# jermp/sshash

Measured on AMD Instinct MI355X. Metric: k-mer Lookups/sec (batched random queries, bit-exact ids), higher is better.
Workload: dtype u64

## Files before the change

sshash_amd/csrc/replica.hpp:

```cpp
#pragma once

#include <algorithm>
#include <atomic>

#include <cstdio>
#include <cstdlib>

#include <hip/hip_runtime.h>

#include <functional>
#include <mutex>
#include <stdexcept>
#include <string>
#include <unordered_map>
#include <vector>

#include "lookup_device.hpp"
#include "mphf_build.hpp"

namespace sshash_amd {

inline void hip_check(hipError_t e, char const* what) {
    if (e != hipSuccess) throw error(error_kind::hip, std::string("HIP error in ") + what + ": " + hipGetErrorString(e));
}
#define HIP_CHECK(x) ::sshash_amd::hip_check((x), #x)

struct device_guard {
    int prev = 0;
    int target;
    explicit device_guard(int dev) : target(dev) {
        HIP_CHECK(hipGetDevice(&prev));
        if (prev != dev) HIP_CHECK(hipSetDevice(dev));
    }
    ~device_guard() {
        if (prev != target) (void)hipSetDevice(prev);
    }
};

struct host_lane {
    hipStream_t stream = nullptr;
    void* pinned = nullptr;
    void* device = nullptr;
    size_t capacity = 0;
};

struct stream_block {
    void* block = nullptr;
    size_t bytes = 0;
    void free_block() {
        if (block) HIP_CHECK(hipFree(block));
        block = nullptr;
        bytes = 0;
    }
    void release() {
        if (block) (void)hipFree(block);
        block = nullptr;
        bytes = 0;
    }
};

template <typename Slot, size_t MAX_STREAMS, size_t MAX_BYTES>
class stream_cache {
public:
    Slot& get(void* stream, size_t bytes, size_t headroom) {
        std::lock_guard<std::mutex> lock(m_mutex);
        auto it = m_slots.try_emplace(stream).first;
        it->second.last_use = ++m_clock;
        Slot& slot = it->second.slot;
        if (slot.bytes >= bytes) return slot;
        slot.free_block();
        const size_t want = bytes + bytes / headroom + 4096;
        size_t held = want;
        for (auto const& kv : m_slots) held += kv.second.slot.bytes;
        while (m_slots.size() > 1 && (m_slots.size() > MAX_STREAMS || held > MAX_BYTES)) {
            auto oldest = m_slots.end();
            for (auto jt = m_slots.begin(); jt != m_slots.end(); ++jt)
                if (jt != it && (oldest == m_slots.end() || jt->second.last_use < oldest->second.last_use)) oldest = jt;
            held -= oldest->second.slot.bytes;
            oldest->second.slot.release();
            m_slots.erase(oldest);
        }
        HIP_CHECK(hipMalloc(&slot.block, want));
        slot.bytes = want;
        return slot;
    }
    void release(void* stream) {
        std::lock_guard<std::mutex> lock(m_mutex);
        auto it = m_slots.find(stream);
        if (it == m_slots.end()) return;
        it->second.slot.release();
        m_slots.erase(it);
    }
    void clear() {
        std::lock_guard<std::mutex> lock(m_mutex);
        for (auto& kv : m_slots) kv.second.slot.release();
        m_slots.clear();
    }

private:
    struct entry {
        Slot slot;
        uint64_t last_use = 0;
    };
    std::mutex m_mutex;
    std::unordered_map<void*, entry> m_slots;
    uint64_t m_clock = 0;
};

struct device_replica {
    int device = -1;
    uint64_t bytes = 0;
    uint64_t bytes_still_to_come = 0;
    dict_view view{};
    skew_part_dev* d_skew = nullptr;
    uint64_t directory_overflowed = 0;
    uint64_t directory_entries = 0;
    uint64_t sk_keys = 0, sk_heavy_keys = 0, sk_heavy_kmers = 0, sk_unplaced = 0, sk_slots_used = 0, sk_bytes = 0;
    uint32_t sk_absent_reason = 1;
    uint64_t sk_histogram[20] = {0};
    std::vector<void*> allocations;
    hipMemPool_t scratch_pool = nullptr;
    void create_scratch_pool() {
        hipMemPoolProps props{};
        props.allocType = hipMemAllocationTypePinned;
        props.handleTypes = hipMemHandleTypeNone;
        props.location.type = hipMemLocationTypeDevice;
        props.location.id = device;
        if (hipMemPoolCreate(&scratch_pool, &props) != hipSuccess) {
            scratch_pool = nullptr;
            (void)hipGetLastError();
            if (std::getenv("SSHASH_AMD_VERBOSE"))
                fprintf(stderr, "[sshash_amd] device %d: no private memory pool (hipMemPoolCreate failed): stream-ordered scratch comes out of the default pool\n", device);
            return;
        }
        uint64_t keep = ~uint64_t(0);
        (void)hipMemPoolSetAttribute(scratch_pool, hipMemPoolAttrReleaseThreshold, &keep);
    }
    void* stream_alloc(size_t bytes, hipStream_t s) const {
        void* p = nullptr;
        if (scratch_pool) HIP_CHECK(hipMallocFromPoolAsync(&p, bytes ? bytes : 8, scratch_pool, s));
        else HIP_CHECK(hipMallocAsync(&p, bytes ? bytes : 8, s));
        return p;
    }

    mutable std::mutex launch_mutex;
    struct stream_scratch : stream_block {
        hipStream_t aux = nullptr;
        hipEvent_t first_done[2] = {nullptr, nullptr};
        hipEvent_t tail_done[2] = {nullptr, nullptr};
        void free_block() {
            if (aux) HIP_CHECK(hipStreamSynchronize(aux));
            stream_block::free_block();
        }
        void release() {
            if (aux) (void)hipStreamSynchronize(aux);
            for (int i = 0; i < 2; ++i) {
                if (first_done[i]) (void)hipEventDestroy(first_done[i]);
                if (tail_done[i]) (void)hipEventDestroy(tail_done[i]);
                first_done[i] = tail_done[i] = nullptr;
            }
            if (aux) (void)hipStreamDestroy(aux);
            aux = nullptr;
            stream_block::release();
        }
    };
    mutable stream_cache<stream_scratch, 16, ~size_t(0)> queue_scratch;
    mutable stream_cache<stream_block, 64, size_t(8) << 30> read_scratch;
    stream_scratch& scratch_for(void* stream, size_t bytes, bool with_aux_stream) const {
        stream_scratch& slot = queue_scratch.get(stream, bytes, 4);
        if (with_aux_stream && !slot.aux) {
            HIP_CHECK(hipStreamCreateWithFlags(&slot.aux, hipStreamNonBlocking));
            for (int i = 0; i < 2; ++i) {
                HIP_CHECK(hipEventCreateWithFlags(&slot.first_done[i], hipEventDisableTiming));
                HIP_CHECK(hipEventCreateWithFlags(&slot.tail_done[i], hipEventDisableTiming));
            }
        }
        return slot;
    }
    void* read_scratch_for(void* stream, size_t bytes) const { return read_scratch.get(stream, bytes, 8).block; }

    void release_stream_scratch(void* stream) const {
        queue_scratch.release(stream);
        read_scratch.release(stream);
    }

    mutable std::mutex lanes_mutex;
    mutable std::vector<host_lane*> idle_lanes;
    host_lane* acquire_lane(size_t bytes) const;
    void release_lane(host_lane* lane) const;

    template <typename T>
    T* put(std::vector<T> const& v) {
        T* d = nullptr;
        const size_t n = (v.empty() ? 1 : v.size()) * sizeof(T);
        HIP_CHECK(hipMalloc(&d, n));
        allocations.push_back(d);
        if (!v.empty()) HIP_CHECK(hipMemcpy(d, v.data(), v.size() * sizeof(T), hipMemcpyHostToDevice));
        bytes += n;
        return d;
    }
    mphf_view put_mphf(mphf_host const& f) {
        mphf_view v = f.view();
        v.parts = put(f.parts);
        v.pilots = put(f.pilots);
        v.free_slots = put(f.free_slots);
        return v;
    }
    device_replica() = default;
    device_replica(device_replica const&) = delete;
    device_replica& operator=(device_replica const&) = delete;
    ~device_replica() {
        if (device < 0) return;
        int prev = 0;
        if (hipGetDevice(&prev) != hipSuccess) return;
        (void)hipSetDevice(device);
        for (void* p : allocations) (void)hipFree(p);
        if (scratch_pool) {
            (void)hipDeviceSynchronize();
            (void)hipMemPoolDestroy(scratch_pool);
        }
        queue_scratch.clear();
        read_scratch.clear();
        for (host_lane* lane : idle_lanes) {
            if (lane->pinned) (void)hipHostFree(lane->pinned);
            if (lane->device) (void)hipFree(lane->device);
            if (lane->stream) (void)hipStreamDestroy(lane->stream);
            delete lane;
        }
        (void)hipSetDevice(prev);
    }
};

struct own_stream {
    device_replica const* rep;
    hipStream_t s = nullptr;
    explicit own_stream(device_replica const* r) : rep(r) { HIP_CHECK(hipStreamCreateWithFlags(&s, hipStreamNonBlocking)); }
    own_stream(own_stream const&) = delete;
    own_stream& operator=(own_stream const&) = delete;
    ~own_stream() {
        (void)hipStreamSynchronize(s);
        rep->release_stream_scratch(s);
        (void)hipStreamDestroy(s);
    }
};

class device_buffers {
public:
    device_buffers() = default;
    device_buffers(device_replica const* rep, hipStream_t s) : m_rep(rep), m_stream(s) {}
    device_buffers(device_buffers const&) = delete;
    device_buffers& operator=(device_buffers const&) = delete;
    ~device_buffers() {
        for (void* p : m_owned) free_one(p);
    }
    template <typename T>
    T* alloc(uint64_t n) {
        const size_t bytes = std::max<uint64_t>(n * sizeof(T), 8);
        void* p = nullptr;
        if (m_rep) p = m_rep->stream_alloc(bytes, m_stream);
        else HIP_CHECK(hipMalloc(&p, bytes));
        m_owned.push_back(p);
        return static_cast<T*>(p);
    }
    void release(void const* p) {
        for (void*& q : m_owned)
            if (q == p) {
                free_one(q);
                q = nullptr;
            }
    }
    void keep(void const* p, device_replica& rep) {
        for (void*& q : m_owned)
            if (q == p) {
                rep.allocations.push_back(q);
                q = nullptr;
            }
    }

private:
    void free_one(void* p) const {
        if (!p) return;
        if (m_rep) (void)hipFreeAsync(p, m_stream);
        else (void)hipFree(p);
    }
    device_replica const* m_rep = nullptr;
    hipStream_t m_stream = nullptr;
    std::vector<void*> m_owned;
};

class engine;

std::vector<int> resident_devices(engine const& eng);

void run_lanes(engine const& eng, std::vector<int> const& devices, size_t bytes, std::function<void(size_t, int, host_lane&)> const& fn,
               std::atomic<bool>* failed = nullptr);

}
```

sshash_amd/csrc/streaming.hip:

```cpp
#include <hip/hip_runtime.h>
#include <sys/stat.h>

#include <algorithm>
#include <atomic>
#include <cstring>
#include <exception>
#include <stdexcept>
#include <thread>

#include "engine.hpp"
#include "hooks.hpp"
#include "reads.hpp"
#include "replica.hpp"

namespace sshash_amd {

namespace {

template <int W, bool CANON>
__device__ __forceinline__ hit_t seed_lookup(dict_view const& d, skew_part_dev const* __restrict__ skew,
                                             kmer_w<W> const& x, kmer_w<W> const& x_rc, minimizer_t mf, minimizer_t mr) {
    if constexpr (CANON) {
        if (mf.value < mr.value) return probe_canonical<W, true>(d, skew, x, x_rc, mf);
        if (mr.value < mf.value) return probe_canonical<W, true>(d, skew, x, x_rc, mr);
        hit_t h = probe_canonical<W, true>(d, skew, x, x_rc, mf);
        if (!h.found) h = probe_canonical<W, true>(d, skew, x, x_rc, mr);
        return h;
    } else {
        hit_t h = probe_regular<W, true>(d, skew, x, mf);
        if (!h.found) {
            const bool mf_found = h.minimizer_found;
            h = probe_regular<W, true>(d, skew, x_rc, mr);
            h.orientation = -1;
            h.minimizer_found = h.minimizer_found || mf_found;
        }
        return h;
    }
}

__device__ __forceinline__ uint64_t wave_sum(uint64_t v) {
    for (int o = 32; o > 0; o >>= 1) v += __shfl_down(v, o, 64);
    return v;
}

__device__ __forceinline__ void block_report(uint64_t c_kmers, uint64_t c_invalid, uint64_t c_negative, uint64_t c_searches,
                                             uint64_t c_extensions, uint64_t* __restrict__ report) {
    __shared__ uint64_t partial[4][5];
    c_kmers = wave_sum(c_kmers);
    c_invalid = wave_sum(c_invalid);
    c_negative = wave_sum(c_negative);
    c_searches = wave_sum(c_searches);
    c_extensions = wave_sum(c_extensions);
    if ((threadIdx.x & 63) == 0) {
        uint64_t* mine = partial[threadIdx.x >> 6];
        mine[0] = c_kmers;
        mine[1] = c_invalid;
        mine[2] = c_negative;
        mine[3] = c_searches;
        mine[4] = c_extensions;
    }
    __syncthreads();
    if (threadIdx.x != 0) return;
    uint64_t t[5];
    for (int j = 0; j < 5; ++j) t[j] = partial[0][j] + partial[1][j] + partial[2][j] + partial[3][j];
    if (t[0] == 0) return;
    atomicAdd(reinterpret_cast<unsigned long long*>(report + 0), (unsigned long long)t[0]);
    atomicAdd(reinterpret_cast<unsigned long long*>(report + 1), (unsigned long long)(t[3] + t[4]));
    atomicAdd(reinterpret_cast<unsigned long long*>(report + 2), (unsigned long long)t[2]);
    atomicAdd(reinterpret_cast<unsigned long long*>(report + 3), (unsigned long long)t[1]);
    atomicAdd(reinterpret_cast<unsigned long long*>(report + 4), (unsigned long long)t[3]);
    atomicAdd(reinterpret_cast<unsigned long long*>(report + 5), (unsigned long long)t[4]);
}


__global__ void __launch_bounds__(256)
stream_pack_kernel(const char* __restrict__ bases, const uint64_t total_bases, uint16_t* __restrict__ packed, uint8_t* __restrict__ okay) {
    const uint64_t t = uint64_t(blockIdx.x) * blockDim.x + threadIdx.x;
    const uint64_t at = 8 * t;
    if (at >= total_bases) return;
    uint64_t v = 0;
    if (at + 8 <= total_bases && ((reinterpret_cast<uintptr_t>(bases) + at) & 7) == 0) {
        v = *reinterpret_cast<const uint64_t*>(bases + at);
    } else {
        for (uint32_t b = 0; b < 8 && at + b < total_bases; ++b) v |= uint64_t(uint8_t(bases[at + b])) << (8 * b);
    }
    uint64_t two = (v >> 1) & 0x0303030303030303ULL;
    two = (two | (two >> 6)) & 0x000F000F000F000FULL;
    two = (two | (two >> 12)) & 0x000000FF000000FFULL;
    two = two | (two >> 24);
    const uint64_t u = v & 0xDFDFDFDFDFDFDFDFULL;
    auto nonzero = [](uint64_t z) { return ((z & 0x7F7F7F7F7F7F7F7FULL) + 0x7F7F7F7F7F7F7F7FULL) | z; };
    uint64_t ok = ~(nonzero(u ^ 0x4141414141414141ULL) & nonzero(u ^ 0x4343434343434343ULL) & nonzero(u ^ 0x4747474747474747ULL) &
                    nonzero(u ^ 0x5454545454545454ULL)) & 0x8080808080808080ULL;
    ok >>= 7;
    ok |= ok >> 7;
    ok |= ok >> 14;
    ok |= ok >> 28;
    packed[t] = uint16_t(two);
    okay[t] = uint8_t(ok);
}

__device__ __forceinline__ uint64_t first_invalid_base(const uint64_t* __restrict__ okay, uint64_t from, uint64_t end) {
    uint64_t p = from;
    while (p < end) {
        const uint64_t bad = ~okay[p >> 6] >> (p & 63u);
        if (bad) {
            p += uint64_t(__builtin_ctzll(bad));
            break;
        }
        p = (p | 63u) + 1;
    }
    return p < end ? p : end;
}

__device__ __forceinline__ uint64_t first_valid_base(const uint64_t* __restrict__ okay, uint64_t from, uint64_t end) {
    uint64_t p = from;
    while (p < end) {
        const uint64_t good = okay[p >> 6] >> (p & 63u);
        if (good) {
            p += uint64_t(__builtin_ctzll(good));
            break;
        }
        p = (p | 63u) + 1;
    }
    return p < end ? p : end;
}

__device__ __forceinline__ uint64_t read_bases32(const uint64_t* __restrict__ packed, uint64_t p) {
    const uint64_t i = p >> 5;
    return funnel_shr(packed[i], packed[i + 1], 2 * (uint32_t(p) & 31u));
}

template <int W>
__device__ __forceinline__ void string_bases32(dict_view const& d, uint64_t p, uint64_t& bases, uint64_t& marks) {
    const uint32_t rel = uint32_t(p) & 31u;
    if constexpr (W == 1) {
        const uint4* A = reinterpret_cast<const uint4*>(d.granules) + 2 * (p >> 5);
        const uint4 q0 = A[0], q1 = A[1];
        bases = funnel_shr(uint64_t(q0.x) | (uint64_t(q0.y) << 32), uint64_t(q0.z) | (uint64_t(q0.w) << 32), 2 * rel);
        marks = (uint64_t(q1.x) | (uint64_t(q1.y) << 32)) >> rel;
    } else {
        const uint4* G = reinterpret_cast<const uint4*>(d.granules) + (p >> 5);
        const uint4 g0 = G[0], g1 = G[1];
        bases = funnel_shr(uint64_t(g0.z) | (uint64_t(g0.w) << 32), uint64_t(g1.z) | (uint64_t(g1.w) << 32), 2 * rel);
        marks = (uint64_t(g0.y) | (uint64_t(g1.y) << 32)) >> rel;
    }
}

struct run_step_t {
    uint64_t s, marks, read;
    uint32_t have;
};

template <int W>
__device__ __forceinline__ run_step_t run_step_load(dict_view const& d, const uint64_t* __restrict__ packed, uint64_t off, bool forward,
                                                    uint64_t b, uint64_t run) {
    run_step_t t;
    const uint64_t top = off - run;
    t.have = forward || top >= 32 ? 32u : uint32_t(top);
    string_bases32<W>(d, forward ? off + d.k + run : top - t.have, t.s, t.marks);
    t.read = read_bases32(packed, b + run);
    return t;
}

__device__ __forceinline__ uint32_t run_step_length(run_step_t const& t, bool forward) {
    const uint64_t along = forward ? t.s : revcomp_word(t.s << ((2 * (32 - t.have)) & 63u));
    const uint64_t diff = along ^ t.read;
    const uint32_t same = diff ? uint32_t(__builtin_ctzll(diff)) >> 1 : 32u;
    const uint32_t gate = forward ? uint32_t(__brev(uint32_t(t.marks))) : uint32_t((t.marks >> 1) << (32 - t.have));
    const uint32_t inside = gate ? uint32_t(__builtin_clz(gate)) : 32u;
    const uint32_t step = same < inside ? same : inside;
    return step < t.have ? step : t.have;
}

template <int W>
__device__ __forceinline__ uint64_t extend_run(dict_view const& d, const uint64_t* __restrict__ packed, uint64_t off, int ori, uint64_t b,
                                               uint64_t room, run_step_t t) {
    const bool forward = ori > 0;
    uint64_t run = 0;
    for (;;) {
        uint64_t step = run_step_length(t, forward);
        if (step > room - run) step = room - run;
        run += step;
        if (step < 32 || run >= room) break;
        t = run_step_load<W>(d, packed, off, forward, b, run);
    }
    return run;
}

__device__ __forceinline__ void row_flush(uint64_t* __restrict__ row, bool partial, uint32_t& c_invalid, uint32_t& c_negative, uint32_t& c_searches,
                                          uint32_t& c_extensions) {
    const uint64_t s = c_searches, e = c_extensions;
    if (partial) {
        row[1] += s + e;
        row[2] += c_negative;
        row[3] += c_invalid;
        row[4] += s;
        row[5] += e;
    } else {
        row[1] = s + e;
        row[2] = c_negative;
        row[3] = c_invalid;
        row[4] = s;
        row[5] = e;
    }
    c_invalid = c_negative = c_searches = c_extensions = 0;
}

#ifndef SSHASH_STREAM_WAVES
#define SSHASH_STREAM_WAVES 5
#endif
enum : int { STREAM_TOTALS = 0, STREAM_ROWS = 1, STREAM_RUN_COUNTS = 2, STREAM_RUN_RECORDS = 3, STREAM_COVER = 4 };

__device__ __forceinline__ void run_record_store(dict_view const& d, run_sink const& sink, const uint64_t* __restrict__ offsets, uint64_t r,
                                                 uint64_t cursor, uint64_t at, uint64_t off, uint32_t sid, int ori, uint64_t n) {
    if (cursor >= sink.capacity || cursor >= sink.run_offsets[r + 1]) return;
    const uint64_t kmer_id = off - uint64_t(sid) * (d.k - 1), in_string = off - d.endpoints[sid];
    const uint32_t read_pos = uint32_t(at - offsets[r]), length = uint32_t(n) | (ori > 0 ? 0u : 0x80000000u);
    uint4* const rec = static_cast<uint4*>(sink.records) + 2 * cursor;
    rec[0] = make_uint4(uint32_t(kmer_id), uint32_t(kmer_id >> 32), sid, 0u);
    rec[1] = make_uint4(uint32_t(in_string), uint32_t(in_string >> 32), read_pos, length);
}

__device__ __forceinline__ void cover_mark(uint64_t* __restrict__ cover, uint64_t lo, uint64_t hi) {
    const uint64_t w0 = lo >> 6, w1 = (hi - 1) >> 6;
    const unsigned long long first = ~0ULL << (lo & 63u), last = ~0ULL >> (63u - (uint32_t(hi - 1) & 63u));
    unsigned long long* const words = reinterpret_cast<unsigned long long*>(cover);
    if (w0 == w1) {
        (void)__hip_atomic_fetch_or(words + w0, first & last, __ATOMIC_RELAXED, __HIP_MEMORY_SCOPE_AGENT);
        return;
    }
    (void)__hip_atomic_fetch_or(words + w0, first, __ATOMIC_RELAXED, __HIP_MEMORY_SCOPE_AGENT);
    for (uint64_t w = w0 + 1; w < w1; ++w) words[w] = ~0ULL;
    (void)__hip_atomic_fetch_or(words + w1, last, __ATOMIC_RELAXED, __HIP_MEMORY_SCOPE_AGENT);
}

__device__ __forceinline__ void cover_mark_run(dict_view const& d, run_sink const& sink, uint64_t off, uint32_t sid, int ori, uint64_t n) {
    const uint64_t kmer_id = off - uint64_t(sid) * (d.k - 1);
    const uint64_t lo = ori > 0 ? kmer_id : kmer_id + 1 - n;
    cover_mark(static_cast<uint64_t*>(sink.records), lo, lo + n);
}

template <int W, bool CANON, bool SK, int MODE>
__global__ void __launch_bounds__(256, SSHASH_STREAM_WAVES)
streaming_run_kernel(const dict_view d, const skew_part_dev* __restrict__ skew, const uint64_t* __restrict__ packed,
                     const uint64_t* __restrict__ okay, const uint64_t* __restrict__ offsets, const uint64_t n_reads,
                     const uint64_t reads_per_wave, const uint32_t move_out_every, uint64_t* __restrict__ report, const run_sink sink) {
    constexpr bool PER_READ = MODE == STREAM_ROWS, COUNT_RUNS = MODE == STREAM_RUN_COUNTS, RECORDS = MODE == STREAM_RUN_RECORDS, COVER = MODE == STREAM_COVER;
    __shared__ uint4 stage[SK ? 4 * 256 : 1];
    uint4* const wave_stage = stage + (SK ? (threadIdx.x >> 6) * 256 : 0);
    __shared__ unsigned long long moved_out[4][5];
    uint32_t c_invalid = 0, c_negative = 0, c_searches = 0, c_extensions = 0;
// ... 288 lines not shown
                        }
                    }
                }
            }
        }
        const bool finishing = live && !walking;
        STAT(st_full, finishing && !settled);
        if (finishing && !settled) {
            const minimizer_t mf = compute_minimizer<W>(x, k, d.m, d.hash_magic);
            const minimizer_t mr = compute_minimizer<W>(x_rc, k, d.m, d.hash_magic);
            if (!SK && neg_unknown_mini && mf.value == prev_f && mr.value == prev_r) {
                found = false;
            } else {
                prev_f = mf.value;
                prev_r = mr.value;
                const hit_t h = seed_lookup<W, CANON>(d, skew, x, x_rc, mf, mr);
                found = h.found;
                off = h.kmer_offset;
                ori = h.orientation;
                if constexpr (RECORDS || COVER) hit_sid = h.string_id;
                neg_unknown_mini = !SK && !h.found && !h.minimizer_found;
            }
        }
        if (finishing) {
            if (found) {
                ++c_searches;
                neg_unknown_mini = false;
                pending = cur + 1 + k <= valid_end;
                if constexpr (COUNT_RUNS) ++n_runs;
                if constexpr (RECORDS) {
                    if (!pending) {
                        run_record_store(d, sink, offsets, wave_first + my_row, cursor, cur, off, hit_sid, ori, 1);
                        ++cursor;
                    }
                }
                if constexpr (COVER) {
                    if (!pending) cover_mark_run(d, sink, off, hit_sid, ori, 1);
                }
            } else {
                ++c_negative;
            }
            ++cur;
        }
    }
#ifdef SSHASH_STREAM_STATS
    const unsigned long long st_neg_kept = wave_sum(st_kept_lane);
    if (lane == 0 && MODE == STREAM_TOTALS) {
        unsigned long long* st = reinterpret_cast<unsigned long long*>(report) + 6;
        atomicAdd(st + 0, st_turns); atomicAdd(st + 1, st_fresh); atomicAdd(st + 2, st_walk); atomicAdd(st + 3, st_ext); atomicAdd(st + 4, st_slot1);
        atomicAdd(st + 5, st_inv); atomicAdd(st + 6, st_idle); atomicAdd(st + 7, st_full); atomicAdd(st + 8, st_neg_kept); atomicAdd(st + 9, st_short);
    }
#endif
    if constexpr (PER_READ) {
        if (my_row != ROW_NONE) row_flush(wave_rows + uint64_t(my_row & ~ROW_PARTIAL) * 6, (my_row & ROW_PARTIAL) != 0, c_invalid, c_negative, c_searches, c_extensions);
    } else if constexpr (!RECORDS) {
        if constexpr (COUNT_RUNS) {
            if (my_row != ROW_NONE) sink.run_offsets[wave_first + my_row] = n_runs;
        }
        const bool first = lane == 0;
        block_report(first ? wave_moved_out[4] : 0, uint64_t(c_invalid) + (first ? wave_moved_out[0] : 0), uint64_t(c_negative) + (first ? wave_moved_out[1] : 0),
                     uint64_t(c_searches) + (first ? wave_moved_out[2] : 0), uint64_t(c_extensions) + (first ? wave_moved_out[3] : 0), report);
    }
}

__global__ void __launch_bounds__(256)
stream_rows_sum_kernel(const uint64_t* __restrict__ rows, const uint64_t n_reads, uint64_t* __restrict__ report) {
    uint64_t c_kmers = 0, c_invalid = 0, c_negative = 0, c_searches = 0, c_extensions = 0;
    const uint64_t stride = uint64_t(gridDim.x) * blockDim.x;
    for (uint64_t r = uint64_t(blockIdx.x) * blockDim.x + threadIdx.x; r < n_reads; r += stride) {
        const uint64_t* row = rows + 6 * r;
        c_kmers += row[0];
        c_negative += row[2];
        c_invalid += row[3];
        c_searches += row[4];
        c_extensions += row[5];
    }
    block_report(c_kmers, c_invalid, c_negative, c_searches, c_extensions, report);
}

constexpr uint32_t SCAN_PER_LANE = 16, SCAN_TILE = 256 * SCAN_PER_LANE;
inline uint64_t scan_tiles(uint64_t n) { return (n + SCAN_TILE - 1) / SCAN_TILE; }

__device__ __forceinline__ uint64_t block_exclusive_scan(uint64_t v, uint64_t& total) {
    __shared__ uint64_t wave_total[4];
    const uint32_t lane = threadIdx.x & 63u, w = threadIdx.x >> 6;
    uint64_t inc = v;
    for (uint32_t o = 1; o < 64; o <<= 1) {
        const uint64_t t = __shfl_up(inc, o, 64);
        if (lane >= o) inc += t;
    }
    __syncthreads();
    if (lane == 63) wave_total[w] = inc;
    __syncthreads();
    uint64_t before = 0;
    total = 0;
    for (uint32_t j = 0; j < 4; ++j) {
        if (j < w) before += wave_total[j];
        total += wave_total[j];
    }
    return before + inc - v;
}

__global__ void __launch_bounds__(256)
scan_tile_sums_kernel(const uint64_t* __restrict__ data, const uint64_t n, uint64_t* __restrict__ sums) {
    const uint64_t base = uint64_t(blockIdx.x) * SCAN_TILE + threadIdx.x * SCAN_PER_LANE;
    uint64_t v = 0;
    for (uint32_t j = 0; j < SCAN_PER_LANE; ++j)
        if (base + j < n) v += data[base + j];
    uint64_t total;
    block_exclusive_scan(v, total);
    if (threadIdx.x == 0) sums[blockIdx.x] = total;
}

__global__ void __launch_bounds__(256)
scan_sums_kernel(uint64_t* __restrict__ sums, const uint64_t tiles) {
    uint64_t carry = 0;
    for (uint64_t at = 0; at < tiles; at += 256) {
        const uint64_t i = at + threadIdx.x;
        const uint64_t v = i < tiles ? sums[i] : 0;
        uint64_t total;
        const uint64_t before = block_exclusive_scan(v, total);
        if (i < tiles) sums[i] = carry + before;
        carry += total;
    }
}

__global__ void __launch_bounds__(256)
scan_apply_kernel(uint64_t* __restrict__ data, const uint64_t n, const uint64_t* __restrict__ sums) {
    const uint64_t base = uint64_t(blockIdx.x) * SCAN_TILE + threadIdx.x * SCAN_PER_LANE;
    uint64_t e[SCAN_PER_LANE], v = 0;
#pragma unroll
    for (uint32_t j = 0; j < SCAN_PER_LANE; ++j) {
        e[j] = base + j < n ? data[base + j] : 0;
        v += e[j];
    }
    uint64_t total;
    uint64_t at = sums[blockIdx.x] + block_exclusive_scan(v, total);
#pragma unroll
    for (uint32_t j = 0; j < SCAN_PER_LANE; ++j) {
        if (base + j < n) data[base + j] = at;
        at += e[j];
    }
}

void exclusive_scan_u64(uint64_t* data, uint64_t n, uint64_t* sums, hipStream_t s) {
    if (n == 0) return;
    const uint64_t tiles = scan_tiles(n);
    hipLaunchKernelGGL(scan_tile_sums_kernel, dim3(uint32_t(tiles)), dim3(256), 0, s, data, n, sums);
    hipLaunchKernelGGL(scan_sums_kernel, dim3(1), dim3(256), 0, s, sums, tiles);
    hipLaunchKernelGGL(scan_apply_kernel, dim3(uint32_t(tiles)), dim3(256), 0, s, data, n, sums);
    HIP_CHECK(hipGetLastError());
}

enum : int { RUNS_COUNT = 1, RUNS_WRITE = 2, RUNS_COVER = 4 };
template <int W, bool CANON>
void launch_streaming_runs(device_replica const* rep, dict_view const& d, char const* bases, uint64_t const* offsets, uint64_t n_reads,
                           uint64_t total_bases, uint64_t* report, hipStream_t s, uint64_t* rows = nullptr ,
                           run_sink sink = run_sink{nullptr, nullptr, 0}, int run_phases = 0) {
    const uint64_t packed_bytes = ((total_bases + 31) / 32 + 3) * 8, okay_bytes = ((total_bases + 63) / 64 + 2) * 8;
    const uint64_t runs_bytes = run_phases ? (scan_tiles(n_reads + 1) + 6) * 8 : 0;
    std::lock_guard<std::mutex> sequence(rep->launch_mutex);
    uint64_t* packed = static_cast<uint64_t*>(rep->read_scratch_for(s, packed_bytes + okay_bytes + runs_bytes));
    uint64_t* okay = packed + packed_bytes / 8;
    uint64_t* scan_sums = okay + okay_bytes / 8;
    if (total_bases) {
        const uint64_t lanes = (total_bases + 7) / 8;
        hipLaunchKernelGGL(stream_pack_kernel, dim3(uint32_t((lanes + 255) / 256)), dim3(256), 0, s, bases, total_bases,
                           reinterpret_cast<uint16_t*>(packed), reinterpret_cast<uint8_t*>(okay));
    }
    const uint64_t max_waves = uint64_t(256) * 4 * SSHASH_STREAM_WAVES;
    uint64_t waves = std::min<uint64_t>(max_waves, std::max<uint64_t>(1, n_reads / (64 * 2)));
    waves = (waves + 3) / 4 * 4;
    const uint64_t reads_per_wave = (n_reads + waves - 1) / waves;
    const dim3 grid(uint32_t(waves / 4)), block(256);
    const uint32_t move_out_every = uint32_t(test_hook_u64("stream_move_out_every", uint64_t(1) << 16, 1, uint64_t(1) << 16));
    if (run_phases) {
        if (run_phases & RUNS_COVER) {
            uint64_t* totals = report;
            if (!totals) {
                totals = scan_sums + scan_tiles(n_reads + 1);
                HIP_CHECK(hipMemsetAsync(totals, 0, 6 * sizeof(uint64_t), s));
            }
            if (d.sk.enabled) hipLaunchKernelGGL((streaming_run_kernel<W, CANON, true, STREAM_COVER>), grid, block, 0, s, d, rep->d_skew, packed, okay, offsets, n_reads, reads_per_wave, move_out_every, totals, sink);
            else hipLaunchKernelGGL((streaming_run_kernel<W, CANON, false, STREAM_COVER>), grid, block, 0, s, d, rep->d_skew, packed, okay, offsets, n_reads, reads_per_wave, move_out_every, totals, sink);
            HIP_CHECK(hipGetLastError());
            return;
        }
        if (reads_per_wave >> 31) throw error(error_kind::argument, "too many reads for one call");
        if (run_phases & RUNS_COUNT) {
            uint64_t* totals = report;
            if (!totals) {
                totals = scan_sums + scan_tiles(n_reads + 1);
                HIP_CHECK(hipMemsetAsync(totals, 0, 6 * sizeof(uint64_t), s));
            }
            if (d.sk.enabled) hipLaunchKernelGGL((streaming_run_kernel<W, CANON, true, STREAM_RUN_COUNTS>), grid, block, 0, s, d, rep->d_skew, packed, okay, offsets, n_reads, reads_per_wave, move_out_every, totals, sink);
            else hipLaunchKernelGGL((streaming_run_kernel<W, CANON, false, STREAM_RUN_COUNTS>), grid, block, 0, s, d, rep->d_skew, packed, okay, offsets, n_reads, reads_per_wave, move_out_every, totals, sink);
            HIP_CHECK(hipGetLastError());
            HIP_CHECK(hipMemsetAsync(sink.run_offsets + n_reads, 0, sizeof(uint64_t), s));
            exclusive_scan_u64(sink.run_offsets, n_reads + 1, scan_sums, s);
        }
        if (run_phases & RUNS_WRITE) {
            if (d.sk.enabled) hipLaunchKernelGGL((streaming_run_kernel<W, CANON, true, STREAM_RUN_RECORDS>), grid, block, 0, s, d, rep->d_skew, packed, okay, offsets, n_reads, reads_per_wave, move_out_every, static_cast<uint64_t*>(nullptr), sink);
            else hipLaunchKernelGGL((streaming_run_kernel<W, CANON, false, STREAM_RUN_RECORDS>), grid, block, 0, s, d, rep->d_skew, packed, okay, offsets, n_reads, reads_per_wave, move_out_every, static_cast<uint64_t*>(nullptr), sink);
            HIP_CHECK(hipGetLastError());
        }
        return;
    }
    if (rows) {
        if (reads_per_wave >> 31) throw error(error_kind::argument, "too many reads for one call");
        if (d.sk.enabled) hipLaunchKernelGGL((streaming_run_kernel<W, CANON, true, STREAM_ROWS>), grid, block, 0, s, d, rep->d_skew, packed, okay, offsets, n_reads, reads_per_wave, move_out_every, rows, sink);
        else hipLaunchKernelGGL((streaming_run_kernel<W, CANON, false, STREAM_ROWS>), grid, block, 0, s, d, rep->d_skew, packed, okay, offsets, n_reads, reads_per_wave, move_out_every, rows, sink);
        HIP_CHECK(hipGetLastError());
        if (report) {
            const uint32_t blocks = uint32_t(std::min<uint64_t>((n_reads + 255) / 256, 1024));
            hipLaunchKernelGGL(stream_rows_sum_kernel, dim3(blocks), dim3(256), 0, s, rows, n_reads, report);
            HIP_CHECK(hipGetLastError());
        }
        return;
    }
    if (d.sk.enabled) hipLaunchKernelGGL((streaming_run_kernel<W, CANON, true, STREAM_TOTALS>), grid, block, 0, s, d, rep->d_skew, packed, okay, offsets, n_reads, reads_per_wave, move_out_every, report, sink);
    else hipLaunchKernelGGL((streaming_run_kernel<W, CANON, false, STREAM_TOTALS>), grid, block, 0, s, d, rep->d_skew, packed, okay, offsets, n_reads, reads_per_wave, move_out_every, report, sink);
    HIP_CHECK(hipGetLastError());
}

}

void engine::streaming_query_device(int device, char const* d_bases, uint64_t const* d_read_offsets, uint64_t n_reads,
                                    uint64_t total_bases, uint64_t* d_report, void* stream) const {
    device_replica const* rep = replica(device);
    if (n_reads == 0) return;
    device_guard guard(device);
    dict_view const& d = rep->view;
    hipStream_t s = hipStream_t(stream);
    const bool wide = d.k > 31;
    if (total_bases == 0) {
        HIP_CHECK(hipMemcpyAsync(&total_bases, d_read_offsets + n_reads, sizeof(uint64_t), hipMemcpyDeviceToHost, s));
        HIP_CHECK(hipStreamSynchronize(s));
        if (total_bases == 0) return;
    }
    if (!wide && !d.canonical) launch_streaming_runs<1, false>(rep, d, d_bases, d_read_offsets, n_reads, total_bases, d_report, s);
    else if (!wide && d.canonical) launch_streaming_runs<1, true>(rep, d, d_bases, d_read_offsets, n_reads, total_bases, d_report, s);
    else if (wide && !d.canonical) launch_streaming_runs<2, false>(rep, d, d_bases, d_read_offsets, n_reads, total_bases, d_report, s);
    else launch_streaming_runs<2, true>(rep, d, d_bases, d_read_offsets, n_reads, total_bases, d_report, s);
}

void engine::streaming_query_per_read_device(int device, char const* d_bases, uint64_t const* d_read_offsets, uint64_t n_reads,
                                             uint64_t total_bases, uint64_t* d_rows, uint64_t* d_report, void* stream) const {
    device_replica const* rep = replica(device);
    if (n_reads == 0) return;
    if (!d_rows) throw error(error_kind::argument, "per-read output pointer is null");
    device_guard guard(device);
    dict_view const& d = rep->view;
    hipStream_t s = hipStream_t(stream);
    const bool wide = d.k > 31;
    if (total_bases == 0) {
        HIP_CHECK(hipMemcpyAsync(&total_bases, d_read_offsets + n_reads, sizeof(uint64_t), hipMemcpyDeviceToHost, s));
        HIP_CHECK(hipStreamSynchronize(s));
        if (total_bases == 0) {
            HIP_CHECK(hipMemsetAsync(d_rows, 0, n_reads * 6 * sizeof(uint64_t), s));
            return;
        }
    }
    if (!wide && !d.canonical) launch_streaming_runs<1, false>(rep, d, d_bases, d_read_offsets, n_reads, total_bases, d_report, s, d_rows);
    else if (!wide && d.canonical) launch_streaming_runs<1, true>(rep, d, d_bases, d_read_offsets, n_reads, total_bases, d_report, s, d_rows);
    else if (wide && !d.canonical) launch_streaming_runs<2, false>(rep, d, d_bases, d_read_offsets, n_reads, total_bases, d_report, s, d_rows);
    else launch_streaming_runs<2, true>(rep, d, d_bases, d_read_offsets, n_reads, total_bases, d_report, s, d_rows);
}

void engine::streaming_runs_device(int device, char const* d_bases, uint64_t const* d_read_offsets, uint64_t n_reads, uint64_t total_bases,
                                   uint64_t* d_run_offsets, void* d_runs, uint64_t runs_capacity, uint64_t* d_report, void* stream) const {
    (void)replica(device);
    if (n_reads == 0 && !d_run_offsets) return;
    if (!d_run_offsets) throw error(error_kind::argument, "run_offsets pointer is null");
    if (!d_runs && runs_capacity) throw error(error_kind::argument, "runs pointer is null");
    streaming_runs_passes(device, d_bases, d_read_offsets, n_reads, total_bases, run_sink{d_run_offsets, d_runs, runs_capacity}, d_report, stream, true,
                          runs_capacity != 0);
}

void engine::streaming_runs_passes(int device, char const* d_bases, uint64_t const* d_read_offsets, uint64_t n_reads, uint64_t total_bases,
                                   run_sink const& sink, uint64_t* d_report, void* stream, bool count, bool write) const {
    device_replica const* rep = replica(device);
    device_guard guard(device);
    dict_view const& d = rep->view;
    hipStream_t s = hipStream_t(stream);
    const bool wide = d.k > 31;
    if (n_reads && total_bases == 0) {
        HIP_CHECK(hipMemcpyAsync(&total_bases, d_read_offsets + n_reads, sizeof(uint64_t), hipMemcpyDeviceToHost, s));
        HIP_CHECK(hipStreamSynchronize(s));
    }
    if (n_reads == 0 || total_bases == 0) {
        if (count) HIP_CHECK(hipMemsetAsync(sink.run_offsets, 0, (n_reads + 1) * sizeof(uint64_t), s));
        return;
    }
    const int phases = (count ? RUNS_COUNT : 0) | (write ? RUNS_WRITE : 0);
    if (!phases) return;
    if (!wide && !d.canonical) launch_streaming_runs<1, false>(rep, d, d_bases, d_read_offsets, n_reads, total_bases, d_report, s, nullptr, sink, phases);
    else if (!wide && d.canonical) launch_streaming_runs<1, true>(rep, d, d_bases, d_read_offsets, n_reads, total_bases, d_report, s, nullptr, sink, phases);
    else if (wide && !d.canonical) launch_streaming_runs<2, false>(rep, d, d_bases, d_read_offsets, n_reads, total_bases, d_report, s, nullptr, sink, phases);
    else launch_streaming_runs<2, true>(rep, d, d_bases, d_read_offsets, n_reads, total_bases, d_report, s, nullptr, sink, phases);
}

void engine::streaming_cover_device(int device, char const* d_bases, uint64_t const* d_read_offsets, uint64_t n_reads, uint64_t total_bases,
                                    uint64_t* d_cover, uint64_t* d_report, void* stream) const {
    device_replica const* rep = replica(device);
    if (n_reads == 0) return;
    if (!d_cover) throw error(error_kind::argument, "cover pointer is null");
    device_guard guard(device);
    dict_view const& d = rep->view;
    hipStream_t s = hipStream_t(stream);
    const bool wide = d.k > 31;
    if (total_bases == 0) {
        HIP_CHECK(hipMemcpyAsync(&total_bases, d_read_offsets + n_reads, sizeof(uint64_t), hipMemcpyDeviceToHost, s));
        HIP_CHECK(hipStreamSynchronize(s));
        if (total_bases == 0) return;
    }
    const run_sink sink{nullptr, d_cover, 0};
    if (!wide && !d.canonical) launch_streaming_runs<1, false>(rep, d, d_bases, d_read_offsets, n_reads, total_bases, d_report, s, nullptr, sink, RUNS_COVER);
    else if (!wide && d.canonical) launch_streaming_runs<1, true>(rep, d, d_bases, d_read_offsets, n_reads, total_bases, d_report, s, nullptr, sink, RUNS_COVER);
    else if (wide && !d.canonical) launch_streaming_runs<2, false>(rep, d, d_bases, d_read_offsets, n_reads, total_bases, d_report, s, nullptr, sink, RUNS_COVER);
    else launch_streaming_runs<2, true>(rep, d, d_bases, d_read_offsets, n_reads, total_bases, d_report, s, nullptr, sink, RUNS_COVER);
}

constexpr uint8_t SQ_VALID = 1, SQ_INVALID = 2, SQ_FIRST = 4;

__device__ __forceinline__ uint32_t nonzero_bytes(uint32_t v) {
    return (((v & 0x7F7F7F7Fu) + 0x7F7F7F7Fu) | v) & 0x80808080u;
}

__global__ void __launch_bounds__(256)
stream_tile_reads_kernel(const uint64_t* __restrict__ offsets, const uint64_t n_reads, const uint64_t first, const uint64_t tiles,
                         uint64_t* __restrict__ tile_read) {
    const uint64_t t = uint64_t(blockIdx.x) * blockDim.x + threadIdx.x;
    if (t >= tiles) return;
    const uint64_t g0 = first + t * 256;
    uint64_t lo = 0, hi = n_reads - 1;
    while (lo < hi) {
        const uint64_t mid = lo + (hi - lo + 1) / 2;
        if (offsets[mid] <= g0) lo = mid;
        else hi = mid - 1;
    }
    tile_read[t] = lo;
}

template <int W>
__global__ void __launch_bounds__(256)
stream_encode_kernel(const char* __restrict__ bases, const uint64_t* __restrict__ offsets, const uint64_t* __restrict__ tile_read, const uint64_t n_reads,
                     const uint64_t total_bases, const uint64_t first, const uint64_t count, const uint32_t k,
                     uint64_t* __restrict__ kmers , uint8_t* __restrict__ flags ) {
    constexpr uint32_t TILE = 256, SPAN = TILE + 64;
    __shared__ uint32_t chars[SPAN / 4 + 2];
    __shared__ uint32_t codes[SPAN / 16 + 4];
    __shared__ uint32_t okay[SPAN / 32 + 4];
    __shared__ uint64_t ends[TILE + 2];
    const uint64_t g0 = first + uint64_t(blockIdx.x) * TILE;
    const uint32_t tid = threadIdx.x;
    const uint64_t r0 = tile_read[blockIdx.x];
    for (uint32_t c = tid; c < SPAN / 4 + 2; c += TILE) {
        const uint64_t at = g0 + 4 * uint64_t(c);
        uint32_t v = 0;
        if (at + 4 <= total_bases && ((reinterpret_cast<uintptr_t>(bases) + at) & 3) == 0) v = *reinterpret_cast<const uint32_t*>(bases + at);
        else
            for (uint32_t b = 0; b < 4; ++b)
                if (at + b < total_bases) v |= uint32_t(uint8_t(bases[at + b])) << (8 * b);
        chars[c] = v;
    }
    __syncthreads();
    for (uint32_t c = tid; c < SPAN / 4 + 2; c += TILE) {
        const uint32_t four = chars[c];
        uint32_t two = (four >> 1) & 0x03030303u;
        two = (two | (two >> 6) | (two >> 12) | (two >> 18)) & 0xFFu;
        reinterpret_cast<uint8_t*>(codes)[c] = uint8_t(two);
    }
    for (uint32_t q = tid; q < SPAN + 64; q += TILE) {
        const uint32_t u = (q < 4 * (SPAN / 4 + 2) ? reinterpret_cast<const uint8_t*>(chars)[q] : 0u) & 0xDFu;
        const uint64_t mask = __ballot(u == 0x41u || u == 0x43u || u == 0x47u || u == 0x54u);
// ... 741 lines not shown
```

Before: 41.10 billion.

## Overlap read packing with streaming lookups via aux-stream pieces and wider pack kernel

Rewrites the base-packing kernel as a grid-stride loop in which each lane loads 16 bytes with a nontemporal vector load and validates bases through a byte-permute lookup. Adds an optional split mode that packs later read ranges on an auxiliary stream while the lookup kernel runs over earlier pieces, joined by events. Split mode is gated by a test hook whose default is zero, so by default only the new pack kernel and the restructured launch code run. The split adds event and stream overhead and cut-boundary logic that must handle k-mers spanning piece edges.

```diff
diff --git a/sshash_amd/csrc/replica.hpp b/sshash_amd/csrc/replica.hpp
--- a/sshash_amd/csrc/replica.hpp
+++ b/sshash_amd/csrc/replica.hpp
@@ -165,7 +165,29 @@
         }
     };
     mutable stream_cache<stream_scratch, 16, ~size_t(0)> queue_scratch;
-    mutable stream_cache<stream_block, 64, size_t(8) << 30> read_scratch;
+    struct read_stream_scratch : stream_block {
+        static constexpr int MAX_AUX_PIECES = 3;
+        hipStream_t aux = nullptr;
+        hipEvent_t entered = nullptr;
+        hipEvent_t packed_done[MAX_AUX_PIECES] = {nullptr, nullptr, nullptr};
+        void free_block() {
+            if (aux) HIP_CHECK(hipStreamSynchronize(aux));
+            stream_block::free_block();
+        }
+        void release() {
+            if (aux) (void)hipStreamSynchronize(aux);
+            if (entered) (void)hipEventDestroy(entered);
+            entered = nullptr;
+            for (hipEvent_t& e : packed_done) {
+                if (e) (void)hipEventDestroy(e);
+                e = nullptr;
+            }
+            if (aux) (void)hipStreamDestroy(aux);
+            aux = nullptr;
+            stream_block::release();
+        }
+    };
+    mutable stream_cache<read_stream_scratch, 64, size_t(8) << 30> read_scratch;
     stream_scratch& scratch_for(void* stream, size_t bytes, bool with_aux_stream) const {
         stream_scratch& slot = queue_scratch.get(stream, bytes, 4);
         if (with_aux_stream && !slot.aux) {
@@ -177,7 +199,15 @@
         }
         return slot;
     }
-    void* read_scratch_for(void* stream, size_t bytes) const { return read_scratch.get(stream, bytes, 8).block; }
+    read_stream_scratch& read_scratch_for(void* stream, size_t bytes, bool with_aux_stream) const {
+        read_stream_scratch& slot = read_scratch.get(stream, bytes, 8);
+        if (with_aux_stream && !slot.aux) {
+            HIP_CHECK(hipStreamCreateWithFlags(&slot.aux, hipStreamNonBlocking));
+            HIP_CHECK(hipEventCreateWithFlags(&slot.entered, hipEventDisableTiming));
+            for (hipEvent_t& e : slot.packed_done) HIP_CHECK(hipEventCreateWithFlags(&e, hipEventDisableTiming));
+        }
+        return slot;
+    }
 
     void release_stream_scratch(void* stream) const {
         queue_scratch.release(stream);
diff --git a/sshash_amd/csrc/streaming.hip b/sshash_amd/csrc/streaming.hip
--- a/sshash_amd/csrc/streaming.hip
+++ b/sshash_amd/csrc/streaming.hip
@@ -73,31 +73,64 @@
 }
 
 
+typedef uint32_t pack_u32x4 __attribute__((ext_vector_type(4)));
+constexpr uint64_t PACK_TO_THE_END = ~uint64_t(0);
+constexpr uint32_t PACK_SLACK_BASES = 96, PACK_LANE_BASES = 16, PACK_LOADS = 2, PACK_TILE_BASES = 256 * PACK_LOADS * PACK_LANE_BASES;
+
+__device__ __forceinline__ uint64_t pack_cut(const uint64_t* __restrict__ offsets, uint64_t r, uint64_t total_bases) {
+    const uint64_t c = (offsets[r] + PACK_SLACK_BASES + 63) & ~uint64_t(63);
+    return c < total_bases ? c : total_bases;
+}
+
+__device__ __forceinline__ void pack_four(uint32_t v, uint32_t& codes, uint32_t& valid) {
+    const uint32_t two = (v >> 1) & 0x03030303u;
+    uint32_t t = (two << 6) | two;
+    t = (t << 12) | t;
+    codes = (t >> 18) & 0xFFu;
+    const uint32_t letters = 0x47544341u;
+    const uint32_t y = (v & 0xDFDFDFDFu) ^ __builtin_amdgcn_perm(letters, letters, two);
+    const uint32_t nonzero = ((y & 0x7F7F7F7Fu) + 0x7F7F7F7Fu) | y;
+    uint32_t ok = ~nonzero & 0x80808080u;
+    ok = (ok << 7) | ok;
+    ok = (ok << 14) | ok;
+    valid = ok >> 28;
+}
+
 __global__ void __launch_bounds__(256)
-stream_pack_kernel(const char* __restrict__ bases, const uint64_t total_bases, uint16_t* __restrict__ packed, uint8_t* __restrict__ okay) {
-    const uint64_t t = uint64_t(blockIdx.x) * blockDim.x + threadIdx.x;
-    const uint64_t at = 8 * t;
-    if (at >= total_bases) return;
-    uint64_t v = 0;
-    if (at + 8 <= total_bases && ((reinterpret_cast<uintptr_t>(bases) + at) & 7) == 0) {
-        v = *reinterpret_cast<const uint64_t*>(bases + at);
-    } else {
-        for (uint32_t b = 0; b < 8 && at + b < total_bases; ++b) v |= uint64_t(uint8_t(bases[at + b])) << (8 * b);
-    }
-    uint64_t two = (v >> 1) & 0x0303030303030303ULL;
-    two = (two | (two >> 6)) & 0x000F000F000F000FULL;
-    two = (two | (two >> 12)) & 0x000000FF000000FFULL;
-    two = two | (two >> 24);
-    const uint64_t u = v & 0xDFDFDFDFDFDFDFDFULL;
-    auto nonzero = [](uint64_t z) { return ((z & 0x7F7F7F7F7F7F7F7FULL) + 0x7F7F7F7F7F7F7F7FULL) | z; };
-    uint64_t ok = ~(nonzero(u ^ 0x4141414141414141ULL) & nonzero(u ^ 0x4343434343434343ULL) & nonzero(u ^ 0x4747474747474747ULL) &
-                    nonzero(u ^ 0x5454545454545454ULL)) & 0x8080808080808080ULL;
-    ok >>= 7;
-    ok |= ok >> 7;
-    ok |= ok >> 14;
-    ok |= ok >> 28;
-    packed[t] = uint16_t(two);
-    okay[t] = uint8_t(ok);
+stream_pack_kernel(const char* __restrict__ bases, const uint64_t total_bases, const uint64_t* __restrict__ offsets, const uint64_t lo_read,
+                   const uint64_t hi_read, uint32_t* __restrict__ packed, uint16_t* __restrict__ okay) {
+    const uint64_t from = lo_read ? pack_cut(offsets, lo_read, total_bases) : 0;
+    const uint64_t to = hi_read != PACK_TO_THE_END ? pack_cut(offsets, hi_read, total_bases) : total_bases;
+    const bool aligned = (reinterpret_cast<uintptr_t>(bases) & 15) == 0;
+    const uint64_t stride = uint64_t(gridDim.x) * PACK_TILE_BASES;
+    for (uint64_t tile = from + uint64_t(blockIdx.x) * PACK_TILE_BASES; tile < to; tile += stride) {
+        pack_u32x4 v[PACK_LOADS];
+#pragma unroll
+        for (uint32_t j = 0; j < PACK_LOADS; ++j) {
+            const uint64_t at = tile + uint64_t(j * 256 + threadIdx.x) * PACK_LANE_BASES;
+            v[j] = pack_u32x4{0u, 0u, 0u, 0u};
+            if (at >= to) continue;
+            if (aligned && at + PACK_LANE_BASES <= total_bases) {
+                v[j] = __builtin_nontemporal_load(reinterpret_cast<const pack_u32x4*>(bases + at));
+            } else {
+                uint32_t w[4] = {0u, 0u, 0u, 0u};
+                for (uint32_t b = 0; b < PACK_LANE_BASES && at + b < total_bases; ++b) w[b >> 2] |= uint32_t(uint8_t(bases[at + b])) << (8 * (b & 3u));
+                v[j] = pack_u32x4{w[0], w[1], w[2], w[3]};
+            }
+        }
+#pragma unroll
+        for (uint32_t j = 0; j < PACK_LOADS; ++j) {
+            const uint64_t at = tile + uint64_t(j * 256 + threadIdx.x) * PACK_LANE_BASES;
+            if (at >= to) continue;
+            uint32_t c0, c1, c2, c3, v0, v1, v2, v3;
+            pack_four(v[j].x, c0, v0);
+            pack_four(v[j].y, c1, v1);
+            pack_four(v[j].z, c2, v2);
+            pack_four(v[j].w, c3, v3);
+            packed[at / PACK_LANE_BASES] = c0 | (c1 << 8) | (c2 << 16) | (c3 << 24);
+            okay[at / PACK_LANE_BASES] = uint16_t(v0 | (v1 << 4) | (v2 << 8) | (v3 << 12));
+        }
+    }
 }
 
 __device__ __forceinline__ uint64_t first_invalid_base(const uint64_t* __restrict__ okay, uint64_t from, uint64_t end) {
@@ -692,6 +725,54 @@
     HIP_CHECK(hipGetLastError());
 }
 
+template <int W, bool CANON, int MODE>
+void launch_run_piece(device_replica const* rep, dict_view const& d, const uint64_t* packed, const uint64_t* okay, uint64_t const* offsets, uint64_t a,
+                      uint64_t b, uint32_t move_out_every, uint64_t* out, run_sink sink, hipStream_t s) {
+    if (b <= a) return;
+    const uint64_t n = b - a;
+    const uint64_t max_waves = uint64_t(256) * 4 * SSHASH_STREAM_WAVES;
+    uint64_t waves = std::min<uint64_t>(max_waves, std::max<uint64_t>(1, n / (64 * 2)));
+    waves = (waves + 3) / 4 * 4;
+    const uint64_t reads_per_wave = (n + waves - 1) / waves;
+    if (MODE != STREAM_TOTALS && MODE != STREAM_COVER && (reads_per_wave >> 31)) throw error(error_kind::argument, "too many reads for one call");
+    const dim3 grid(uint32_t(waves / 4)), block(256);
+    if (MODE == STREAM_ROWS && out) out += 6 * a;
+    if (sink.run_offsets) sink.run_offsets += a;
+    if (d.sk.enabled) hipLaunchKernelGGL((streaming_run_kernel<W, CANON, true, MODE>), grid, block, 0, s, d, rep->d_skew, packed, okay, offsets + a, n, reads_per_wave, move_out_every, out, sink);
+    else hipLaunchKernelGGL((streaming_run_kernel<W, CANON, false, MODE>), grid, block, 0, s, d, rep->d_skew, packed, okay, offsets + a, n, reads_per_wave, move_out_every, out, sink);
+    HIP_CHECK(hipGetLastError());
+}
+
+constexpr uint32_t STREAM_SPLIT_PIECES = 2, STREAM_SPLIT_AUX_BLOCKS = 256, PACK_MAX_BLOCKS = 256 * 8;
+
+struct split_plan {
+    uint64_t cut[device_replica::read_stream_scratch::MAX_AUX_PIECES + 2];
+    uint32_t pieces;
+};
+inline split_plan stream_split_plan(uint64_t n_reads) {
+    const uint64_t first = test_hook_u64("stream_overlap_reads", 0, 0, ~uint64_t(0));
+    const uint32_t most = uint32_t(test_hook_u64("stream_overlap_pieces", STREAM_SPLIT_PIECES, 2, device_replica::read_stream_scratch::MAX_AUX_PIECES + 1));
+    split_plan plan;
+    plan.cut[0] = 0;
+    plan.pieces = 0;
+    uint64_t size = first;
+    while (first && plan.pieces + 1 < most && size < n_reads - plan.cut[plan.pieces]) {
+        plan.cut[plan.pieces + 1] = plan.cut[plan.pieces] + size;
+        ++plan.pieces;
+        size = size > n_reads / 4 ? n_reads : 4 * size;
+    }
+    plan.cut[++plan.pieces] = n_reads;
+    return plan;
+}
+
+inline void launch_pack(char const* bases, uint64_t total_bases, uint64_t const* offsets, uint64_t lo_read, uint64_t hi_read, uint64_t* packed, uint64_t* okay,
+                        uint32_t max_blocks, hipStream_t s) {
+    const uint64_t tiles = (total_bases + PACK_TILE_BASES - 1) / PACK_TILE_BASES;
+    hipLaunchKernelGGL(stream_pack_kernel, dim3(uint32_t(std::min<uint64_t>(tiles, max_blocks))), dim3(256), 0, s, bases, total_bases, offsets, lo_read, hi_read,
+                       reinterpret_cast<uint32_t*>(packed), reinterpret_cast<uint16_t*>(okay));
+    HIP_CHECK(hipGetLastError());
+}
+
 enum : int { RUNS_COUNT = 1, RUNS_WRITE = 2, RUNS_COVER = 4 };
 template <int W, bool CANON>
 void launch_streaming_runs(device_replica const* rep, dict_view const& d, char const* bases, uint64_t const* offsets, uint64_t n_reads,
@@ -699,68 +780,54 @@
                            run_sink sink = run_sink{nullptr, nullptr, 0}, int run_phases = 0) {
     const uint64_t packed_bytes = ((total_bases + 31) / 32 + 3) * 8, okay_bytes = ((total_bases + 63) / 64 + 2) * 8;
     const uint64_t runs_bytes = run_phases ? (scan_tiles(n_reads + 1) + 6) * 8 : 0;
+    const split_plan plan = stream_split_plan(n_reads);
+    const bool split = plan.pieces > 1 && total_bases != 0;
     std::lock_guard<std::mutex> sequence(rep->launch_mutex);
-    uint64_t* packed = static_cast<uint64_t*>(rep->read_scratch_for(s, packed_bytes + okay_bytes + runs_bytes));
+    device_replica::read_stream_scratch& scratch = rep->read_scratch_for(s, packed_bytes + okay_bytes + runs_bytes, split);
+    uint64_t* packed = static_cast<uint64_t*>(scratch.block);
     uint64_t* okay = packed + packed_bytes / 8;
     uint64_t* scan_sums = okay + okay_bytes / 8;
-    if (total_bases) {
-        const uint64_t lanes = (total_bases + 7) / 8;
-        hipLaunchKernelGGL(stream_pack_kernel, dim3(uint32_t((lanes + 255) / 256)), dim3(256), 0, s, bases, total_bases,
-                           reinterpret_cast<uint16_t*>(packed), reinterpret_cast<uint8_t*>(okay));
-    }
-    const uint64_t max_waves = uint64_t(256) * 4 * SSHASH_STREAM_WAVES;
-    uint64_t waves = std::min<uint64_t>(max_waves, std::max<uint64_t>(1, n_reads / (64 * 2)));
-    waves = (waves + 3) / 4 * 4;
-    const uint64_t reads_per_wave = (n_reads + waves - 1) / waves;
-    const dim3 grid(uint32_t(waves / 4)), block(256);
     const uint32_t move_out_every = uint32_t(test_hook_u64("stream_move_out_every", uint64_t(1) << 16, 1, uint64_t(1) << 16));
-    if (run_phases) {
-        if (run_phases & RUNS_COVER) {
-            uint64_t* totals = report;
-            if (!totals) {
-                totals = scan_sums + scan_tiles(n_reads + 1);
-                HIP_CHECK(hipMemsetAsync(totals, 0, 6 * sizeof(uint64_t), s));
-            }
-            if (d.sk.enabled) hipLaunchKernelGGL((streaming_run_kernel<W, CANON, true, STREAM_COVER>), grid, block, 0, s, d, rep->d_skew, packed, okay, offsets, n_reads, reads_per_wave, move_out_every, totals, sink);
-            else hipLaunchKernelGGL((streaming_run_kernel<W, CANON, false, STREAM_COVER>), grid, block, 0, s, d, rep->d_skew, packed, okay, offsets, n_reads, reads_per_wave, move_out_every, totals, sink);
-            HIP_CHECK(hipGetLastError());
-            return;
-        }
-        if (reads_per_wave >> 31) throw error(error_kind::argument, "too many reads for one call");
-        if (run_phases & RUNS_COUNT) {
-            uint64_t* totals = report;
-            if (!totals) {
-                totals = scan_sums + scan_tiles(n_reads + 1);
-                HIP_CHECK(hipMemsetAsync(totals, 0, 6 * sizeof(uint64_t), s));
-            }
-            if (d.sk.enabled) hipLaunchKernelGGL((streaming_run_kernel<W, CANON, true, STREAM_RUN_COUNTS>), grid, block, 0, s, d, rep->d_skew, packed, okay, offsets, n_reads, reads_per_wave, move_out_every, totals, sink);
-            else hipLaunchKernelGGL((streaming_run_kernel<W, CANON, false, STREAM_RUN_COUNTS>), grid, block, 0, s, d, rep->d_skew, packed, okay, offsets, n_reads, reads_per_wave, move_out_every, totals, sink);
-            HIP_CHECK(hipGetLastError());
-            HIP_CHECK(hipMemsetAsync(sink.run_offsets + n_reads, 0, sizeof(uint64_t), s));
-            exclusive_scan_u64(sink.run_offsets, n_reads + 1, scan_sums, s);
-        }
-        if (run_phases & RUNS_WRITE) {
-            if (d.sk.enabled) hipLaunchKernelGGL((streaming_run_kernel<W, CANON, true, STREAM_RUN_RECORDS>), grid, block, 0, s, d, rep->d_skew, packed, okay, offsets, n_reads, reads_per_wave, move_out_every, static_cast<uint64_t*>(nullptr), sink);
-            else hipLaunchKernelGGL((streaming_run_kernel<W, CANON, false, STREAM_RUN_RECORDS>), grid, block, 0, s, d, rep->d_skew, packed, okay, offsets, n_reads, reads_per_wave, move_out_every, static_cast<uint64_t*>(nullptr), sink);
-            HIP_CHECK(hipGetLastError());
-        }
-        return;
-    }
-    if (rows) {
-        if (reads_per_wave >> 31) throw error(error_kind::argument, "too many reads for one call");
-        if (d.sk.enabled) hipLaunchKernelGGL((streaming_run_kernel<W, CANON, true, STREAM_ROWS>), grid, block, 0, s, d, rep->d_skew, packed, okay, offsets, n_reads, reads_per_wave, move_out_every, rows, sink);
-        else hipLaunchKernelGGL((streaming_run_kernel<W, CANON, false, STREAM_ROWS>), grid, block, 0, s, d, rep->d_skew, packed, okay, offsets, n_reads, reads_per_wave, move_out_every, rows, sink);
+    const bool per_read = !run_phases && rows;
+    uint64_t* totals = report;
+    if (!totals && (run_phases & (RUNS_COVER | RUNS_COUNT))) {
+        totals = scan_sums + scan_tiles(n_reads + 1);
+        HIP_CHECK(hipMemsetAsync(totals, 0, 6 * sizeof(uint64_t), s));
+    }
+    auto first_pass = [&](uint64_t a, uint64_t b) {
+        if (run_phases & RUNS_COVER) launch_run_piece<W, CANON, STREAM_COVER>(rep, d, packed, okay, offsets, a, b, move_out_every, totals, sink, s);
+        else if (run_phases & RUNS_COUNT) launch_run_piece<W, CANON, STREAM_RUN_COUNTS>(rep, d, packed, okay, offsets, a, b, move_out_every, totals, sink, s);
+        else if (run_phases & RUNS_WRITE) launch_run_piece<W, CANON, STREAM_RUN_RECORDS>(rep, d, packed, okay, offsets, a, b, move_out_every, nullptr, sink, s);
+        else if (rows) launch_run_piece<W, CANON, STREAM_ROWS>(rep, d, packed, okay, offsets, a, b, move_out_every, rows, sink, s);
+        else launch_run_piece<W, CANON, STREAM_TOTALS>(rep, d, packed, okay, offsets, a, b, move_out_every, report, sink, s);
+    };
+    if (!split) {
+        if (total_bases) launch_pack(bases, total_bases, offsets, 0, PACK_TO_THE_END, packed, okay, PACK_MAX_BLOCKS, s);
+        first_pass(0, n_reads);
+    } else {
+        const uint32_t aux_blocks = uint32_t(test_hook_u64("stream_overlap_blocks", STREAM_SPLIT_AUX_BLOCKS, 1, PACK_MAX_BLOCKS));
+        HIP_CHECK(hipEventRecord(scratch.entered, s));
+        HIP_CHECK(hipStreamWaitEvent(scratch.aux, scratch.entered, 0));
+        launch_pack(bases, total_bases, offsets, 0, plan.cut[1], packed, okay, PACK_MAX_BLOCKS, s);
+        for (uint32_t i = 1; i < plan.pieces; ++i) {
+            launch_pack(bases, total_bases, offsets, plan.cut[i], i + 1 == plan.pieces ? PACK_TO_THE_END : plan.cut[i + 1], packed, okay, aux_blocks, scratch.aux);
+            HIP_CHECK(hipEventRecord(scratch.packed_done[i - 1], scratch.aux));
+        }
+        for (uint32_t i = 0; i < plan.pieces; ++i) {
+            if (i) HIP_CHECK(hipStreamWaitEvent(s, scratch.packed_done[i - 1], 0));
+            first_pass(plan.cut[i], plan.cut[i + 1]);
+        }
+    }
+    if (run_phases & RUNS_COUNT) {
+        HIP_CHECK(hipMemsetAsync(sink.run_offsets + n_reads, 0, sizeof(uint64_t), s));
+        exclusive_scan_u64(sink.run_offsets, n_reads + 1, scan_sums, s);
+        if (run_phases & RUNS_WRITE) launch_run_piece<W, CANON, STREAM_RUN_RECORDS>(rep, d, packed, okay, offsets, 0, n_reads, move_out_every, nullptr, sink, s);
+    }
+    if (per_read && report) {
+        const uint32_t blocks = uint32_t(std::min<uint64_t>((n_reads + 255) / 256, 1024));
+        hipLaunchKernelGGL(stream_rows_sum_kernel, dim3(blocks), dim3(256), 0, s, rows, n_reads, report);
         HIP_CHECK(hipGetLastError());
-        if (report) {
-            const uint32_t blocks = uint32_t(std::min<uint64_t>((n_reads + 255) / 256, 1024));
-            hipLaunchKernelGGL(stream_rows_sum_kernel, dim3(blocks), dim3(256), 0, s, rows, n_reads, report);
-            HIP_CHECK(hipGetLastError());
-        }
-        return;
-    }
-    if (d.sk.enabled) hipLaunchKernelGGL((streaming_run_kernel<W, CANON, true, STREAM_TOTALS>), grid, block, 0, s, d, rep->d_skew, packed, okay, offsets, n_reads, reads_per_wave, move_out_every, report, sink);
-    else hipLaunchKernelGGL((streaming_run_kernel<W, CANON, false, STREAM_TOTALS>), grid, block, 0, s, d, rep->d_skew, packed, okay, offsets, n_reads, reads_per_wave, move_out_every, report, sink);
-    HIP_CHECK(hipGetLastError());
+    }
 }
 
 }
```

Result: slower. 39.91 billion (-2.9%).
